# KLab/YAIK

Hardware: AMD Instinct MI355X
Metric: Mpix/s tile encode (alpha reject + 7 gradient passes + 8x8 range quant), 8K RGBA (higher is better)
Workload: dtype u8/int32 (+f32 mode-selection sums)

## Files before the change

yaik_amd/csrc/yk_encode2.hip:

```cpp
#include "yk_common.h"
#include "yk_curves.h"
#include "yk_device.h"
#include <mutex>

__constant__ float c_curve2[6][16] = YK_CURVE_TABLE;

#define LS YK_LSTRIDE
#ifdef YK_TEST_HOOKS
#define YK2_ABLATE(bit) ((P.ablate & (bit)) != 0)
#else
#define YK2_ABLATE(bit) false
#endif

__device__ __forceinline__ int y2_byte(uint32_t w, int ch) { return (w >> (8 * ch)) & 255; }
__device__ __forceinline__ uint32_t y2_absdiff(uint32_t a, uint32_t b) { uint32_t r; asm("v_sad_u32 %0, %1, %2, 0" : "=v"(r) : "v"(a), "v"(b)); return r; }
__device__ __forceinline__ int y2_round6(int v) { return (v & ~3) | (v >> 6); }
__device__ __forceinline__ int y2_round6p(int v) { v = min(v + 1, 255); return (v & ~3) | (v >> 6); }

typedef short y2s2 __attribute__((ext_vector_type(2)));
typedef unsigned short y2u2 __attribute__((ext_vector_type(2)));
__device__ __forceinline__ y2u2 y2_u2(uint32_t w) { return __builtin_bit_cast(y2u2, w); }
__device__ __forceinline__ y2s2 y2_s2(y2u2 v) { return __builtin_bit_cast(y2s2, v); }
__device__ __forceinline__ y2u2 y2_splat(int v) { const unsigned short t = (unsigned short)v; return (y2u2){ t, t }; }
__device__ __forceinline__ y2s2 y2_splats(int v) { const short t = (short)v; return (y2s2){ t, t }; }
// ... 377 lines not shown
    const int lane = pass.lane;
    const unsigned long long viable = y2_viable<SX, SY>(pass, cov) & ~evaluated;
    evaluated = 0ULL;
    if (viable == 0ULL) return;
    YK2_STAT(kPassId * 10 + 0, 1); YK2_STAT(kPassId * 10 + 8, __popcll(y2_spread<NX, NY>(viable)));
    if (y2_compact_sweep<SX, SY>(pass, viable, cov, evaluated)) return;
    const unsigned long long accept = y2_full_pass<SX, SY, SMOOTH>(pass, viable);
    if (accept == 0ULL) return;
    YK2_STAT(kPassId * 10 + 6, 1);
    y2_accept<SX, SY>(pass, cov, accept);
}

#define YK2_QROWS 258
#define YK2_QR0 32
#define YK2_QNR 224
#define YK2_QBYTES ((size_t)YK2_QNR * YK2_QROWS * 16)
#define YK2_RCPBYTES ((size_t)256 * sizeof(float))
#define YK2_DEFN1 224
#define YK2_DEFBYTES ((size_t)225 * YK2_DEFN1 * 4)
#define YK2_TABBYTES (YK2_QBYTES + YK2_RCPBYTES + YK2_DEFBYTES)
typedef _Float16 y2h2 __attribute__((ext_vector_type(2)));
__device__ __forceinline__ uint32_t y2_f16_bits(int n) { const _Float16 h = (_Float16)(float)n; return (uint32_t)__builtin_bit_cast(unsigned short, h); }
__global__ void yk_qtab_kernel(uint4* tab) {
    __shared__ int K[6][16];
    const int R = YK2_QR0 + (int)blockIdx.x, t = threadIdx.x;
    if (t < 96) { const int m = t >> 4, i = t & 15; K[m][i] = __float2int_rz(__fmul_rn(c_curve2[m][i], (float)R)); }
    __syncthreads();
    if (t < YK2_QROWS) {
        const int o = t - 2;
        uint32_t md[6], idx = 0;
        for (int m = 0; m < 6; m++) {
            const int cnt = m < 3 ? 16 : 8;
            int best = 1 << 30, bi = 0;
            for (int n = 0; n < cnt; n++) { const int d = abs(K[m][n] - o); if (d < best) { best = d; bi = n; } }
            best = min(best, 255);
            md[m] = y2_f16_bits(best);
            idx |= (uint32_t)bi << (4 * m);
        }
        tab[(size_t)blockIdx.x * YK2_QROWS + t] = make_uint4(md[0] | (md[1] << 16), md[2] | (md[3] << 16), md[4] | (md[5] << 16), idx);
    }
}
struct Y2TileDef { int base, BN, dist, R; };
__device__ __forceinline__ Y2TileDef y2_tile_def(const int min_, const int d8) {
    Y2TileDef d;
    d.base = (min_ * 63 + 112) / 224;
    d.BN = (d.base * 224) / 63;
    const int scale = 223 - d.BN;
    const int dnum = (d8 - 32) * 127 + (scale - 1);
    d.dist = (scale < 0) ? -dnum : dnum / scale;
    d.R = (d.dist * scale) / 127 + 32;
    return d;
}
__global__ void yk_deftab_kernel(uint32_t* tab) {
    const int min_ = blockIdx.x, d8 = 32 + (int)threadIdx.x;
    const Y2TileDef d = y2_tile_def(min_, d8);
    const int R = min(max(d.R, YK2_QR0), YK2_QR0 + YK2_QNR - 1);
    const uint32_t rowBase = (uint32_t)((R - YK2_QR0) * YK2_QROWS + 2 - d.BN + 256);
    tab[min_ * YK2_DEFN1 + (int)threadIdx.x] = rowBase | (((((uint32_t)d.dist & 255u) << 7) | ((uint32_t)d.base & 255u)) << 16);
}

__global__ void yk_selftest_qtab_kernel(const uint4* tab, const uint32_t* deftab, int* mismatches) {
    const int mn = blockIdx.x, mx = threadIdx.x;
    if (mx < mn) return;
    const int min_ = min(mn, 224);
    int diff = mx - min_; if (diff < 16) diff = 16;
    const int d8 = max(diff, 32);
    const Y2TileDef d = y2_tile_def(min_, d8);
    const int BN = d.BN, R = d.R;
    int bad = 0;
    if (R < YK2_QR0 || R >= YK2_QR0 + YK2_QNR || mn - BN < -2) { atomicAdd(mismatches, 1); return; }
    {
        const uint32_t e = deftab[min_ * YK2_DEFN1 + (d8 - 32)];
        if ((e & 0xFFFFu) != (uint32_t)((R - YK2_QR0) * YK2_QROWS + 2 - BN + 256)) bad++;
        if ((e >> 16) != ((((uint32_t)d.dist & 255u) << 7) | ((uint32_t)d.base & 255u))) bad++;
    }
    for (int m = 0; m < 6; m++) {
        const int cnt = m < 3 ? 16 : 8;
        int L[16];
        for (int i = 0; i < cnt; i++) {
            L[i] = __float2int_rz(__fadd_rn((float)BN, __fmul_rn(c_curve2[m][i], (float)R)));
            if (L[i] != BN + __float2int_rz(__fmul_rn(c_curve2[m][i], (float)R))) bad++;
        }
        for (int v = mn; v <= mx; v++) {
            int best = 1 << 30, bi = 0;
            for (int n = 0; n < cnt; n++) { const int dd = abs(L[n] - v); if (dd < best) { best = dd; bi = n; } }
            const uint4 row = tab[(size_t)(R - YK2_QR0) * YK2_QROWS + (v - BN + 2)];
            const uint32_t w = m < 2 ? row.x : (m < 4 ? row.y : row.z);
            const uint32_t hb = (m & 1) ? (w >> 16) : (w & 0xFFFFu);
            const int ix = (row.w >> (4 * m)) & 15;
            if (hb != y2_f16_bits(best) || ix != bi) bad++;
        }
    }
    if (bad) atomicAdd(mismatches, bad);
}

#define YK2_RUN 16
template <int K> __device__ __forceinline__ uint32_t y2_writelane_k(uint32_t v, uint32_t old) { asm("v_writelane_b32 %0, %1, %2" : "+v"(old) : "s"(v), "n"(K)); return old; }
__device__ __forceinline__ uint32_t y2_writelane(uint32_t v, int k, uint32_t old) {
    switch (k) {
        case 0: return y2_writelane_k<0>(v, old); case 1: return y2_writelane_k<1>(v, old); case 2: return y2_writelane_k<2>(v, old);
        case 3: return y2_writelane_k<3>(v, old); case 4: return y2_writelane_k<4>(v, old); case 5: return y2_writelane_k<5>(v, old);
        case 11: return y2_writelane_k<11>(v, old); default: return y2_writelane_k<12>(v, old);
    }
}
#ifdef YK2_TIMING
__device__ unsigned long long g_y2_times[65536 * 16];
#define YK2_PROBE(i) do { if ((i) == 0 && lane == 0 && unit < 65536) { g_y2_times[(size_t)unit * 16 + 10] = 0; g_y2_times[(size_t)unit * 16 + 11] = 0; g_y2_times[(size_t)unit * 16 + 12] = y2_t_entry; g_y2_times[(size_t)unit * 16 + 13] = ((unsigned long long)y2_xcc << 32) | y2_hwid; } if (lane == 0 && unit < 65536) { g_y2_times[(size_t)unit * 16 + 2 * (i)] = __builtin_amdgcn_s_memtime(); g_y2_times[(size_t)unit * 16 + 2 * (i) + 1] = __builtin_amdgcn_s_memrealtime(); } } while (0)
extern "C" int yk_debug_wave_times(unsigned long long* out) { return (int)hipMemcpyFromSymbol(out, HIP_SYMBOL(g_y2_times), sizeof(g_y2_times)); }
#else
#define YK2_PROBE(i) do { } while (0)
#endif
#define YK2_LUTW 84
#ifndef YK2_WIN
#define YK2_WIN 16
#endif
#ifndef YK2_PREF
#define YK2_PREF 8
#endif
#ifndef YK2_RVWIN
#define YK2_RVWIN 8
#endif

#define Y2_QUAD_X 0xB1
#define Y2_QUAD_Y 0x4E
template <int CTRL> __device__ __forceinline__ int y2_quad(int v) { return __builtin_amdgcn_update_dpp(v, v, CTRL, 0xF, 0xF, true); }
template <int CTRL> __device__ __forceinline__ float y2_quad(float v) { return __int_as_float(y2_quad<CTRL>(__float_as_int(v))); }
template <int FIRST> __device__ __forceinline__ void y2_quad_sums(float (&t)[6]) {
#define Y2_QX(i) "v_add_f32_dpp %" #i ", %" #i ", %" #i " quad_perm:[1,0,3,2] row_mask:0xf bank_mask:0xf\n\t"
#define Y2_QY(i) "v_add_f32_dpp %" #i ", %" #i ", %" #i " quad_perm:[2,3,0,1] row_mask:0xf bank_mask:0xf\n\t"
    if (FIRST == 0)
        asm volatile("s_nop 1\n\t" Y2_QX(0) Y2_QX(1) Y2_QX(2) Y2_QX(3) Y2_QX(4) Y2_QX(5) Y2_QY(0) Y2_QY(1) Y2_QY(2) Y2_QY(3) Y2_QY(4) Y2_QY(5)
                     : "+v"(t[0]), "+v"(t[1]), "+v"(t[2]), "+v"(t[3]), "+v"(t[4]), "+v"(t[5]));
    else
        asm volatile("s_nop 1\n\t" Y2_QX(0) Y2_QX(1) Y2_QX(2) Y2_QY(0) Y2_QY(1) Y2_QY(2) : "+v"(t[3]), "+v"(t[4]), "+v"(t[5]));
#undef Y2_QX
#undef Y2_QY
}
__device__ __forceinline__ float y2_row16_sum(float x) {
    x = __fadd_rn(x, y2_quad<Y2_QUAD_X>(x));
    x = __fadd_rn(x, y2_quad<Y2_QUAD_Y>(x));
    x = __fadd_rn(x, __int_as_float(__builtin_amdgcn_update_dpp(0, __float_as_int(x), 0x141, 0xF, 0xF, true)));
    x = __fadd_rn(x, __int_as_float(__builtin_amdgcn_update_dpp(0, __float_as_int(x), 0x140, 0xF, 0xF, true)));
    return x;
}
__device__ __forceinline__ uint32_t y2_byte_x4(uint32_t w, int ch) {
    uint32_t r; const uint32_t two = 2u;
    if (ch == 0) asm("v_lshlrev_b32_sdwa %0, %1, %2 dst_sel:DWORD dst_unused:UNUSED_PAD src0_sel:DWORD src1_sel:BYTE_0" : "=v"(r) : "v"(two), "v"(w));
    else if (ch == 1) asm("v_lshlrev_b32_sdwa %0, %1, %2 dst_sel:DWORD dst_unused:UNUSED_PAD src0_sel:DWORD src1_sel:BYTE_1" : "=v"(r) : "v"(two), "v"(w));
    else asm("v_lshlrev_b32_sdwa %0, %1, %2 dst_sel:DWORD dst_unused:UNUSED_PAD src0_sel:DWORD src1_sel:BYTE_2" : "=v"(r) : "v"(two), "v"(w));
    return r;
}
__device__ __forceinline__ void y2_fma_lo(float& acc, uint32_t h, float w) { asm volatile("v_fma_mix_f32 %0, %1, %2, %0 op_sel_hi:[1,0,0]" : "+v"(acc) : "v"(h), "v"(w)); }
__device__ __forceinline__ void y2_fma_hi(float& acc, uint32_t h, float w) { asm volatile("v_fma_mix_f32 %0, %1, %2, %0 op_sel:[1,0,0] op_sel_hi:[1,0,0]" : "+v"(acc) : "v"(h), "v"(w)); }
__device__ __forceinline__ uint32_t y2_pack3(int r, int g, int b) {
    return __builtin_amdgcn_perm((uint32_t)b, __builtin_amdgcn_perm((uint32_t)g, (uint32_t)r, 0x0C0C0400u), 0x0C040100u);
}

template <bool WANT_DST, bool MODE3>
__global__ __launch_bounds__(64, 4) void yk_encode2_kernel(const YkEncodeParams P) {
    constexpr int kStart = MODE3 ? 3 : 0;
    constexpr int kPixWords = 17 * LS, kLutWords = WANT_DST ? 16 * YK2_LUTW : 0;
    __shared__ __attribute__((aligned(16))) uint32_t s_mem[kPixWords > kLutWords ? kPixWords : kLutWords];
    uint32_t* const s_pix = s_mem;
    uint32_t (*const s_lut)[YK2_LUTW] = reinterpret_cast<uint32_t (*)[YK2_LUTW]>(s_mem);
    __shared__ uint32_t s_bm[24];
    __shared__ uint8_t s_list[64];
    __shared__ __attribute__((aligned(16))) float s_curve[WANT_DST ? 6 : 1][16];
    __shared__ __attribute__((aligned(16))) float s_rcp[256];
    __shared__ __attribute__((aligned(16))) uint32_t s_aux[432];
    uint32_t* const s_lat = s_aux;
    float (*const s_chain)[68] = reinterpret_cast<float (*)[68]>(s_aux);
    float* const s_err = reinterpret_cast<float*>(s_aux + 408);
    __shared__ uint32_t s_range[3 * 64];
    __shared__ __attribute__((aligned(16))) uint32_t s_sp[3 * 4 * 8 + 3 * 4 * 16];

    uint32_t* const s_tile = s_aux + 416;
    __shared__ uint32_t s_iwTest[WANT_DST ? 1024 : 1];
    uint32_t* const s_iw = WANT_DST ? s_iwTest : s_mem;
    uint32_t* const s_park = WANT_DST ? s_iwTest : s_sp;
    static_assert(WANT_DST || kPixWords >= 1024, "index words need 4 KB");

    const int lane = threadIdx.x;
    __builtin_amdgcn_s_setprio(3);
#ifdef YK2_TIMING
    const unsigned long long y2_t_entry = __builtin_amdgcn_s_memrealtime();
    const unsigned y2_hwid = __builtin_amdgcn_s_getreg((4 << 0) | (0 << 6) | (31 << 11)), y2_xcc = __builtin_amdgcn_s_getreg((20 << 0) | (0 << 6) | (31 << 11));
#endif
    typedef const __attribute__((address_space(4))) YkEncodeParams* Y2ParamPtr;
    auto strip = [&](const int slot, const int xcd, const int lane, Y2ParamPtr const Pp) {
    const __attribute__((address_space(4))) YkEncodeParams& P = *Pp;
    const int nBf = P.xBB64 * P.yBB64, nB = nBf * P.nFrames;
    const int grp = slot / (YK2_RUN * 4);
    const int unit = (grp * 8 + ((xcd + grp) & 7)) * (YK2_RUN * 4) + (slot - grp * (YK2_RUN * 4));
    int L = unit >> 2; const int wave = unit & 3;
    const bool spare = L >= nB;
    L = spare ? 0 : L;
    const uint32_t frU = yk_udiv((uint32_t)L, P.divNBf.mul, P.divNBf.shift);
    L -= (int)frU * nBf;
    const size_t fr = frU;
    const int32_t* const pl0 = P.plane[0] + fr * P.fs.plane; const int32_t* const pl1 = P.plane[1] + fr * P.fs.plane; const int32_t* const pl2 = P.plane[2] + fr * P.fs.plane;
    const int BY = (int)yk_udiv((uint32_t)L, P.divXBB64.mul, P.divXBB64.shift), BX = L - BY * P.xBB64;
    const int w = P.w, h = P.h;
    const int mt0 = (BY * 4 + wave) * P.mtW + BX * 4;

    YK2_PROBE(0);
    if (lane < 24) s_bm[lane] = 0;
    typedef uint32_t y2_u32x2 __attribute__((ext_vector_type(2)));
    typedef int32_t y2_i32x4 __attribute__((ext_vector_type(4)));
    y2_u32x2 keep8; y2_i32x4 bnd;
    {
        const int g4 = (lane & 15) * 4, r0 = lane >> 4;
        const int gx = BX * 64 + g4;
        const bool inX = gx + 3 < w;
        const int gxc = min(gx, w - 4);
        const int gyS = BY * 64 + wave * 16;
        const int gyB = min(gyS, P.hAvail - 1);
        const size_t rowBase = (size_t)gyB * (size_t)P.strideElems;
        const char* const b0 = reinterpret_cast<const char*>(pl0 + rowBase);
        const char* const b1 = reinterpret_cast<const char*>(pl1 + rowBase);
        const char* const b2 = reinterpret_cast<const char*>(pl2 + rowBase);
        int4 R[4], G[4], B[4];
#pragma unroll
        for (int k = 0; k < 4; k++) {
            const int rel = min(gyS + r0 + 4 * k, P.hAvail - 1) - gyB;
            const uint32_t off = (uint32_t)(rel * P.strideElems + gxc) * 4u;
            R[k] = *reinterpret_cast<const int4*>(b0 + off);
            G[k] = *reinterpret_cast<const int4*>(b1 + off);
            B[k] = *reinterpret_cast<const int4*>(b2 + off);
        }
        int4 Rb, Gb, Bb;
        {
            const int rel = min(gyS + 16, P.hAvail - 1) - gyB;
            const uint32_t off = (uint32_t)(rel * P.strideElems + gxc) * 4u;
            Rb = *reinterpret_cast<const int4*>(b0 + off);
            Gb = *reinterpret_cast<const int4*>(b1 + off);
            Bb = *reinterpret_cast<const int4*>(b2 + off);
        }
        uint32_t hcol;
        const int hr = min(max(lane - 32, 0), 16);
        {
            const int rel = min(gyS + hr, P.hAvail - 1) - gyB;
            const uint32_t off = (uint32_t)(rel * P.strideElems + min(BX * 64 + 64, w - 1)) * 4u;
            hcol = y2_pack3(*reinterpret_cast<const int32_t*>(b0 + off), *reinterpret_cast<const int32_t*>(b1 + off), *reinterpret_cast<const int32_t*>(b2 + off));
        }
        const float4 rc4 = *reinterpret_cast<const float4*>(P.qtab + YK2_QBYTES + (size_t)lane * 16);
        const uint4* const orow = P.outTab + (wave * YK2_OT_ROWS + (lane & (YK2_OT_ROWS - 1))) * 2;
        const uint4 ta = orow[0], tb = orow[1];
        {
            const bool rowIn = BY * 64 + wave * 16 < h;
            const uintptr_t args = reinterpret_cast<uintptr_t>(Pp);
            const uintptr_t kpIn = reinterpret_cast<uintptr_t>(P.keep) + fr * P.fs.keep + (uintptr_t)(mt0 & ~3);
            const uintptr_t bpIn = reinterpret_cast<uintptr_t>(P.bounds) + fr * 64;
            const uintptr_t kp = (P.keep != nullptr && rowIn) ? kpIn : args, bp = P.bounds != nullptr ? bpIn : args;
            asm volatile("s_load_dwordx2 %0, %2, 0x0\n\ts_load_dwordx4 %1, %3, 0x0" : "=&s"(keep8), "=&s"(bnd) : "s"(kp), "s"(bp));
        }

        __builtin_amdgcn_s_setprio(0);
        if (spare) return;
        {
            const uint32_t frT = frU + P.outFrame0;
            const uint32_t o = ta.x + frT * ta.y + (uint32_t)BX * ta.z + (uint32_t)BY * ta.w;
            s_park[lane] = ((uint32_t)BX < tb.x && (uint32_t)BY < tb.y) ? o : YK2_OT_NONE;
            s_park[64 + lane] = tb.z;
        }
        uint4 o[4], ob;
#pragma unroll
        for (int k = 0; k < 4; k++) {
            o[k] = make_uint4(y2_pack3(R[k].x, G[k].x, B[k].x), y2_pack3(R[k].y, G[k].y, B[k].y), y2_pack3(R[k].z, G[k].z, B[k].z), y2_pack3(R[k].w, G[k].w, B[k].w));
            *reinterpret_cast<uint4*>(&s_pix[(r0 + 4 * k) * LS + g4]) = o[k];
        }
        ob = make_uint4(y2_pack3(Rb.x, Gb.x, Bb.x), y2_pack3(Rb.y, Gb.y, Bb.y), y2_pack3(Rb.z, Gb.z, Bb.z), y2_pack3(Rb.w, Gb.w, Bb.w));
        if (lane < 16) *reinterpret_cast<uint4*>(&s_pix[16 * LS + g4]) = ob;
        if (BX * 64 + 64 > w) {
            if (!inX) {
#pragma unroll
                for (int k = 0; k < 4; k++) *reinterpret_cast<uint4*>(&s_pix[(r0 + 4 * k) * LS + g4]) = make_uint4(o[k].w, o[k].w, o[k].w, o[k].w);
                if (lane < 16) *reinterpret_cast<uint4*>(&s_pix[16 * LS + g4]) = make_uint4(ob.w, ob.w, ob.w, ob.w);
            }
        }
        if (lane >= 32 && lane <= 48) s_pix[hr * LS + 64] = hcol;
        *reinterpret_cast<float4*>(&s_rcp[lane * 4]) = rc4;

    }
    asm volatile("s_waitcnt lgkmcnt(0)" : "+s"(keep8), "+s"(bnd));
    __syncthreads();
    YK2_PROBE(1);

    const int q = lane >> 4, cx = y2_cell_x(lane & 15), cy = y2_cell_y(lane & 15);
    const int bxCell = q * 16 + cx * 4, byCell = wave * 16 + cy * 4;
    const int gxCell = BX * 64 + bxCell, gyCell = BY * 64 + byCell;
    const int lcell = (cy * 4) * LS + bxCell;
    const int lat = cy * 17 + q * 4 + cx;
    const bool mtIn = (BX * 64 + q * 16 < w) && (BY * 64 + wave * 16 < h);

    uint32_t pw[16];
#pragma unroll
    for (int r = 0; r < 4; r++) {
        const uint4 t = *reinterpret_cast<const uint4*>(&s_pix[lcell + r * LS]);
        pw[r * 4 + 0] = t.x; pw[r * 4 + 1] = t.y; pw[r * 4 + 2] = t.z; pw[r * 4 + 3] = t.w;
    }

    unsigned long long cov = 0ULL;
    unsigned long long evaluated = 0ULL;
    {
        bool dead = !mtIn;
        {
            const int lim = 4 * P.rejectFactor + 1;
            const y2u2 rb0 = y2_u2(pw[0] & 0x00FF00FFu), rb1 = y2_u2(pw[1] & 0x00FF00FFu), rb2 = y2_u2(pw[2] & 0x00FF00FFu), rb3 = y2_u2(pw[3] & 0x00FF00FFu);
            const y2u2 ga = y2_u2(__builtin_amdgcn_perm(pw[1], pw[0], 0x0C050C01u)), gb = y2_u2(__builtin_amdgcn_perm(pw[2], pw[1], 0x0C050C01u)),
                       gc = y2_u2(__builtin_amdgcn_perm(pw[3], pw[2], 0x0C050C01u));
            const y2u2 l2 = y2_splat(lim);
            const y2u2 u1 = rb0 + rb2 - rb1 - rb1 + l2, u2 = rb1 + rb3 - rb2 - rb2 + l2, ug = ga + gc - gb - gb + l2;
            const y2u2 um = __builtin_elementwise_max(__builtin_elementwise_max(u1, u2), ug);
            dead |= __builtin_bit_cast(uint32_t, __builtin_elementwise_sub_sat(um, y2_splat(2 * lim))) != 0u;
        }
        const unsigned long long deadLanes = __ballot(dead);
        YK2_STAT(75, 1); YK2_STAT(76, ~deadLanes == 0ULL ? 1 : 0); YK2_STAT(77, __popcll(deadLanes));
        const bool stripInside = (BX * 64 + 64 <= w) && (BY * 64 + wave * 16 + 16 <= h);
        if (~deadLanes != 0ULL && !YK2_ABLATE(2)) {
            auto latticePoint = [&](const int idx) {
                const int lr = (idx * 241) >> 12, lc = idx - lr * 17;
                const uint32_t raw = s_pix[(lr * 4) * LS + lc * 4];
                const uint32_t r6 = (raw & 0x00FCFCFCu) | ((raw >> 6) & 0x00030303u);
                const uint32_t z = (raw & 0x007F7F7Fu) + 0x00010101u;
                const uint32_t inc = (z ^ (raw & 0x00808080u)) | (((z & raw & 0x00808080u) >> 7) * 255u);
                const uint32_t p6 = (inc & 0x00FCFCFCu) | ((inc >> 6) & 0x00030303u);
                s_lat[0 * YK2_LATN + idx] = __builtin_amdgcn_perm(r6, raw, 0x0C040C00u);
                s_lat[1 * YK2_LATN + idx] = __builtin_amdgcn_perm(r6, raw, 0x0C050C01u);
                s_lat[2 * YK2_LATN + idx] = __builtin_amdgcn_perm(r6, raw, 0x0C060C02u);
                s_lat[3 * YK2_LATN + idx] = __builtin_amdgcn_perm(p6, p6, 0x0C010C00u);
                s_lat[4 * YK2_LATN + idx] = __builtin_amdgcn_perm(p6, p6, 0x0C020C02u);
            };
            latticePoint(lane);
            if (lane < YK2_LATN - 64) latticePoint(lane + 64);
            __syncthreads();
            y2s2 rg[16], bb[8];
#pragma unroll
            for (int k = 0; k < 16; k++) rg[k] = y2_rg(pw[k]);
#pragma unroll
            for (int k = 0; k < 8; k++) bb[k] = y2_bb(pw[2 * k], pw[2 * k + 1]);
            const Y2Pass S = { s_lat, lat, cx, cy, rg, bb, deadLanes, stripInside, gxCell, gyCell, w, h, P.rejectFactor, s_bm, bxCell, byCell, s_pix, s_list, s_range, lane };
            if (deadLanes == 0ULL) y2_grad_pass<4, 4, true>(S, cov, evaluated);
            else y2_grad_pass<4, 4>(S, cov, evaluated);
            if (~(cov | deadLanes) != 0ULL) {
                y2_grad_pass<4, 3>(S, cov, evaluated);
                y2_grad_pass<3, 4>(S, cov, evaluated);
                y2_grad_pass<3, 3>(S, cov, evaluated);
                y2_grad_pass<3, 2>(S, cov, evaluated);
                y2_grad_pass<2, 3>(S, cov, evaluated);
                y2_grad_pass<2, 2>(S, cov, evaluated);
            }
#pragma unroll
            for (int r = 0; r < 4; r++) {
                const uint4 t = *reinterpret_cast<const uint4*>(&s_pix[lcell + r * LS]);
                pw[r * 4 + 0] = t.x; pw[r * 4 + 1] = t.y; pw[r * 4 + 2] = t.z; pw[r * 4 + 3] = t.w;
            }
        }
    }
    const int mtIdx = mt0 + q;
    __syncthreads();
    YK2_PROBE(2);
    uint8_t* const small = P.small;
    const uint32_t tabOff = s_park[lane], tabSel = s_park[64 + lane];
    const uint32_t tabVal = (s_bm[tabSel & 31u] >> ((tabSel >> 8) & 31u)) & (~0u >> (tabSel >> 16));
    uint32_t off32 = (uint32_t)lane - 8u < 5u ? tabOff : ~0u;
    uint32_t val32 = (uint32_t)lane - 8u < 3u ? tabVal : 0u;
    {
        if ((uint32_t)lane - 1u < 3u) *(small + tabOff) = (uint8_t)tabVal;
        const unsigned long long t = ((cov >> 2) ^ cov) & 0x0C0C0C0C0C0C0C0CULL;
        const unsigned long long covRM = cov ^ t ^ (t << 2);
        uint32_t off16 = ((lane & 15) == 0 && mtIn) ? P.oCov + (frU * (uint32_t)P.fs.coverage + (uint32_t)mtIdx) * 2u : ~0u;
        uint32_t val16 = (uint32_t)((covRM >> (q * 16)) & 0xFFFFULL);
        if ((uint32_t)lane - 4u < 3u) { off16 = tabOff; val16 = tabVal; }
        if (off16 != ~0u) *reinterpret_cast<uint16_t*>(small + off16) = (uint16_t)val16;
        if (P.pixCache != nullptr) {
            const bool cellIn = (gxCell < w) && (gyCell < h);
            if (cellIn && !((cov >> lane) & 1ULL)) {
                const uint32_t strip = (uint32_t)((BY * 4 + wave) * P.xBB64 + BX);
                uint4* dstp = P.pixCache + (size_t)strip * 256 + lane;
#pragma unroll
                for (int r = 0; r < 4; r++) dstp[r * 64] = make_uint4(pw[r * 4 + 0], pw[r * 4 + 1], pw[r * 4 + 2], pw[r * 4 + 3]);
            }
        }
    }
    YK2_PROBE(3);
    int cxB = 0, cyB = 0, cw = w, chh = P.fullH, discard = 1;
    if (P.bounds != nullptr) {
        const int b0 = bnd.x, b1 = bnd.y, b2 = bnd.z, b3 = bnd.w;
        discard = (b0 == 0 && b1 == 0 && b2 == w && b3 == P.fullH) ? 1 : 0;
        cxB = (b0 >> 3) << 3; cyB = (b1 >> 3) << 3;
        cw = (((b2 + 7) >> 3) << 3) - cxB; chh = (((b3 + 7) >> 3) << 3) - cyB;
    }
    const int cxl = cx & 1, cyl = cy & 1;
    const int tgx = gxCell - cxl * 4, tgyl = gyCell - cyl * 4, tgy = tgyl + P.y0;
    const bool tileIn = (tgx + 8 <= w) && (tgyl + 8 <= h);
    const bool part = tileIn && tgx >= cxB && tgx < cxB + cw && tgy >= cyB && tgy < cyB + chh && (tgx + 8 <= cw) && (tgy + 8 <= chh);
    const uint32_t keep4 = (uint32_t)((((unsigned long long)keep8.y << 32) | keep8.x) >> (8 * (mt0 & 3)));
    const bool keepMT = (P.keep == nullptr) || discard || (mtIn && ((keep4 >> (8 * q)) & 0xFFu) != 0u);
    const bool tileLive = part && keepMT;
    const int l00 = lane & ~3;
    const uint32_t quadN = (uint32_t)((~cov) >> l00) & 15u;
    const int v00 = (int)(quadN & 1u), v01 = (int)((quadN >> 2) & 1u);
    const bool valid = tileLive && ((quadN >> (lane & 3)) & 1u);
    const int nTop = __popc(quadN & 3u), nBot = __popc(quadN >> 2);
    const int tileIdx = (tgyl >> 3) * P.tilesW + (tgx >> 3);
    const size_t T8 = (size_t)P.tilesW * P.tilesH;
    const int tw = lane >> 2;
    const bool writer = ((lane & 3) == 0) && tileIn;
    const unsigned long long validMask = __ballot(valid);
    const bool fullTiles = !WANT_DST && __ballot(tileLive && quadN != 15u && quadN != 0u) == 0ULL;

    {
        const int n16 = (tileLive && !YK2_ABLATE(1)) ? (nTop + nBot) : 0;
        if ((P.tilesW & 7) == 0) {
            if (validMask != 0ULL) {
#pragma unroll
                for (int r = 0; r < 2; r++) {
                    const bool mine = writer && ((cy >> 1) == r);
                    const unsigned long long b0 = __ballot(mine && (n16 & 1)), b1 = __ballot(mine && (n16 & 2)), b2 = __ballot(mine && (n16 & 4));
                    const unsigned long long bd = __ballot(mine && n16 > 0);
                    val32 = y2_writelane((uint32_t)(__popcll(b0) + 2 * __popcll(b1) + 4 * __popcll(b2)) | ((uint32_t)__popcll(bd) << 16), 11 + r, val32);
                }
            }
        } else if (writer && n16 > 0) {
            uint32_t* const blockCntP = P.blockCnt + fr * P.fs.blockN;
            atomicAdd(&blockCntP[((size_t)tileIdx >> 10) * 2], 16u * (uint32_t)n16);
            atomicAdd(&blockCntP[((size_t)tileIdx >> 10) * 2 + 1], 1u);
        }
        if (off32 != ~0u) *reinterpret_cast<uint32_t*>(small + off32) = val32;
    }

    YK2_STAT(70, validMask != 0ULL ? 1 : 0); YK2_STAT(74, __popcll(validMask));
    { const int nv = __popcll(validMask); YK2_STAT(120 + (nv == 0 ? 0 : nv <= 4 ? 1 : nv <= 8 ? 2 : nv <= 16 ? 3 : nv <= 32 ? 4 : nv < 64 ? 5 : 6), 1); (void)nv; }
    uint32_t defs01 = 0u, defs2c = 0u;
    if (validMask != 0ULL && !YK2_ABLATE(1)) {
        uint8_t* const slotsP = P.slots + fr * P.fs.slots;
        uint32_t* lut = &s_lut[WANT_DST ? tw : 0][0];
        if (WANT_DST) {
            s_curve[lane >> 4][lane & 15] = c_curve2[lane >> 4][lane & 15];
            if (lane < 32) s_curve[4 + (lane >> 4)][lane & 15] = c_curve2[4 + (lane >> 4)][lane & 15];
        }
        const int j4 = lane & 3;
        const int nValidLanes = __popcll(validMask);
        const bool spread = nValidLanes <= 4 && !WANT_DST;
        const int vRank = (int)__builtin_amdgcn_mbcnt_hi((uint32_t)(validMask >> 32), __builtin_amdgcn_mbcnt_lo((uint32_t)validMask, 0u));
        uint32_t slotOff[4];
#pragma unroll
        for (int r = 0; r < 4; r++) {
            const int yIn = cyl * 4 + r;
            const int pos = (yIn < 4) ? (yIn * 4 * nTop + (cxl ? 4 * v00 : 0))
                                      : (16 * nTop + (yIn - 4) * 4 * nBot + (cxl ? 4 * v01 : 0));
            slotOff[r] = (uint32_t)tileIdx * (uint32_t)YK_SLOT + (uint32_t)(pos >> 1);
        }
        int tmn[3], tmx[3];
        {
            y2u2 mnRB = y2_splat(0xFFFF), mxRB = y2_splat(0), mnG = y2_splat(0xFFFF), mxG = y2_splat(0);
            if (valid) {
#pragma unroll
                for (int k = 0; k < 16; k += 2) {
                    const y2u2 a = y2_u2(pw[k] & 0x00FF00FFu), b = y2_u2(pw[k + 1] & 0x00FF00FFu), g = y2_u2(__builtin_amdgcn_perm(pw[k + 1], pw[k], 0x0C050C01u));
                    if (k == 0) { mnRB = __builtin_elementwise_min(a, b); mxRB = __builtin_elementwise_max(a, b); mnG = g; mxG = g; }
                    else {
                        mnRB = __builtin_elementwise_min(__builtin_elementwise_min(mnRB, a), b); mxRB = __builtin_elementwise_max(__builtin_elementwise_max(mxRB, a), b);
                        mnG = __builtin_elementwise_min(mnG, g); mxG = __builtin_elementwise_max(mxG, g);
                    }
                }
            }
            tmn[0] = (int)mnRB.x; tmn[2] = (int)mnRB.y; tmx[0] = (int)mxRB.x; tmx[2] = (int)mxRB.y;
            tmn[1] = min((int)mnG.x, (int)mnG.y); tmx[1] = max((int)mxG.x, (int)mxG.y);
#pragma unroll
            for (int p = 0; p < 3; p++) {
                tmn[p] = min(tmn[p], y2_quad<Y2_QUAD_X>(tmn[p])); tmx[p] = max(tmx[p], y2_quad<Y2_QUAD_X>(tmx[p]));
                tmn[p] = min(tmn[p], y2_quad<Y2_QUAD_Y>(tmn[p])); tmx[p] = max(tmx[p], y2_quad<Y2_QUAD_Y>(tmx[p]));
            }
        }
        const uint32_t* const defTab = reinterpret_cast<const uint32_t*>(P.qtab + YK2_QBYTES + YK2_RCPBYTES);
        uint32_t tdef[3];
#pragma unroll
        for (int p = 0; p < 3; p++) {
            const int none = tmn[p] > 255;
            const int mn = none ? 0 : tmn[p], mx = none ? 0 : tmx[p];
            const int min_ = min(mn, 224);
            const int d8 = max(mx - min_, 32);
            tdef[p] = defTab[(uint32_t)(min_ * YK2_DEFN1 + d8 - 32)];
            s_range[p * 64 + lane] = (uint32_t)mn | ((uint32_t)mx << 8);
        }
        const uint8_t* const qrows = P.qtab - (size_t)256 * 16;
        if (spread && !YK2_ABLATE(4)) {
            if (valid) s_list[vRank] = (uint8_t)lane;
            __builtin_amdgcn_fence(__ATOMIC_RELEASE, "wavefront"); __builtin_amdgcn_wave_barrier(); __builtin_amdgcn_fence(__ATOMIC_ACQUIRE, "wavefront");
            const int spI = lane >> 4, spK = lane & 15;
            const bool spAct = spI < nValidLanes;
            const int spSrc = (int)s_list[spAct ? spI : 0];
            const int sq = spSrc >> 4, scx = y2_cell_x(spSrc & 15), scy = y2_cell_y(spSrc & 15);
            const uint32_t spx = s_pix[(scy * 4 + (spK >> 2)) * LS + sq * 16 + scx * 4 + (spK & 3)];
#pragma unroll
            for (int p = 0; p < 3; p++) {
                const uint32_t q16s = (uint32_t)__builtin_amdgcn_ds_bpermute(spSrc << 2, (int)((tdef[p] & 0xFFFFu) << 4));
                float t6[6] = { 0.0f, 0.0f, 0.0f, 0.0f, 0.0f, 0.0f };
                if (spAct) {
                    const uint32_t v4 = y2_byte_x4(spx, p);
                    const uint4 row = *reinterpret_cast<const uint4*>(qrows + (size_t)((v4 << 2) + q16s));
                    const float rv = *reinterpret_cast<const float*>(reinterpret_cast<const char*>(s_rcp) + v4);
                    if (!MODE3) { y2_fma_lo(t6[0], row.x, rv); y2_fma_hi(t6[1], row.x, rv); y2_fma_lo(t6[2], row.y, rv); }
                    y2_fma_hi(t6[3], row.y, rv); y2_fma_lo(t6[4], row.z, rv); y2_fma_hi(t6[5], row.z, rv);
                    s_sp[96 + (p * 4 + spI) * 16 + spK] = row.w;
                }
#pragma unroll
                for (int m = kStart; m < 6; m++) {
                    const float tot = y2_row16_sum(t6[m]);
                    if (spK == 0) s_sp[(p * 4 + spI) * 8 + m] = __float_as_uint(tot);
                }
            }
            __builtin_amdgcn_fence(__ATOMIC_RELEASE, "wavefront"); __builtin_amdgcn_wave_barrier(); __builtin_amdgcn_fence(__ATOMIC_ACQUIRE, "wavefront");
        }
        uint4 win[16];
        auto issueRows = [&](const int pl, const int k0, const int k1) {
            if (valid && !spread && !YK2_ABLATE(4)) {
                const uint32_t q16 = (tdef[pl] & 0xFFFFu) << 4;
                {
#pragma unroll
                    for (int k = k0; k < k1; k++) {
                        const uint32_t v4 = y2_byte_x4(pw[k], pl);
                        win[k] = *reinterpret_cast<const uint4*>(qrows + (size_t)((v4 << 2) + q16));
                    }
                }
            }
        };
        issueRows(0, 0, YK2_PREF);
#pragma unroll
        for (int p = 0; p < 3; p++) {
            const uint32_t qrow16 = (tdef[p] & 0xFFFFu) << 4;
            float sm[6] = { 0.0f, 0.0f, 0.0f, 0.0f, 0.0f, 0.0f };
            issueRows(p, YK2_PREF, 16);
            if (valid && !spread && !YK2_ABLATE(4)) {
                float rvw[YK2_RVWIN];
                auto issueRcp = [&](const int k, float& rv) { rv = *reinterpret_cast<const float*>(reinterpret_cast<const char*>(s_rcp) + y2_byte_x4(pw[k], p)); };
#pragma unroll
                for (int k = 0; k < YK2_RVWIN; k++) issueRcp(k, rvw[k]);
#pragma unroll
                for (int k = 0; k < 16; k++) {
                    __builtin_amdgcn_sched_barrier(0);
                    const uint4 row = win[k]; const float rv = rvw[k % YK2_RVWIN];
                    if (!MODE3) { y2_fma_lo(sm[0], row.x, rv); y2_fma_hi(sm[1], row.x, rv); y2_fma_lo(sm[2], row.y, rv); }
                    y2_fma_hi(sm[3], row.y, rv); y2_fma_lo(sm[4], row.z, rv); y2_fma_hi(sm[5], row.z, rv);
                    s_iw[k * 64 + lane] = row.w;
                    if (k + YK2_RVWIN < 16) issueRcp(k + YK2_RVWIN, rvw[k % YK2_RVWIN]);
                }
                __builtin_amdgcn_sched_barrier(0);
            }
            if (spread && valid && !YK2_ABLATE(4)) {
#pragma unroll
                for (int m = kStart; m < 6; m++) sm[m] = __uint_as_float(s_sp[(p * 4 + vRank) * 8 + m]);
#pragma unroll
                for (int k4 = 0; k4 < 4; k4++) {
                    const uint4 iw4 = *reinterpret_cast<const uint4*>(&s_sp[96 + (p * 4 + vRank) * 16 + k4 * 4]);
                    s_iw[(k4 * 4 + 0) * 64 + lane] = iw4.x; s_iw[(k4 * 4 + 1) * 64 + lane] = iw4.y; s_iw[(k4 * 4 + 2) * 64 + lane] = iw4.z; s_iw[(k4 * 4 + 3) * 64 + lane] = iw4.w;
                }
            }
            if (p < 2) issueRows(p + 1, 0, YK2_PREF);
            float tm[6] = { sm[0], sm[1], sm[2], sm[3], sm[4], sm[5] };
            y2_quad_sums<kStart>(tm);
            int bestMode = kStart; float bestT = tm[kStart];
            bool near = false;
#pragma unroll
            for (int m = kStart + 1; m < 6; m++) {
                const float t = tm[m];
                const float lo = fminf(t, bestT), hi = fmaxf(t, bestT);
                near |= !(__fmul_rn(lo, 1.00002f) < hi);
                bestMode = (t <= bestT) ? m : bestMode;
                bestT = lo;
            }
            bool amb = false;
            uint32_t ties = 0;
            if (__ballot(near && tileLive) != 0ULL) {
                int bm = kStart; float bt = tm[kStart];
#pragma unroll
                for (int m = kStart + 1; m < 6; m++) {
                    const float t = tm[m];
                    const float lo = fminf(t, bt), hi = fmaxf(t, bt);
                    const bool eq = (t == bt);
                    amb |= !eq && !(__fmul_rn(lo, 1.00002f) < hi);
                    if (eq && t != 0.0f) ties |= (1u << m) | ((uint32_t)bm << (8 + 3 * m));
                    bm = (t <= bt) ? m : bm;
                    bt = lo;
                }
            }
            if (__ballot(ties != 0u && tileLive) != 0ULL) {
                YK2_STAT(73, 1);
                const uint32_t tr = s_range[p * 64 + lane];
                const uint32_t mn = tr & 255u, mx = tr >> 8;
                const uint32_t va = min(mn + (uint32_t)j4, mx), vb = min(mn + 4u + (uint32_t)j4, mx);
                const uint4 ra = *reinterpret_cast<const uint4*>(qrows + (size_t)((va << 4) + qrow16));
                const uint4 rb = *reinterpret_cast<const uint4*>(qrows + (size_t)((vb << 4) + qrow16));
                const uint32_t rxa = __builtin_amdgcn_alignbit(ra.x, ra.x, 16), rya = __builtin_amdgcn_alignbit(ra.y, ra.y, 16), rza = __builtin_amdgcn_alignbit(ra.z, ra.z, 16);
                const uint32_t rxb = __builtin_amdgcn_alignbit(rb.x, rb.x, 16), ryb = __builtin_amdgcn_alignbit(rb.y, rb.y, 16), rzb = __builtin_amdgcn_alignbit(rb.z, rb.z, 16);
                uint32_t acc[9] = { (ra.x ^ rxa) | (rb.x ^ rxb),
                                    (ra.y ^ rya) | (rb.y ^ ryb),
                                    (ra.z ^ rza) | (rb.z ^ rzb),
                                    (ra.x ^ ra.y) | (rb.x ^ rb.y),
                                    (ra.x ^ ra.z) | (rb.x ^ rb.z),
                                    (ra.y ^ ra.z) | (rb.y ^ rb.z),
                                    (ra.x ^ rya) | (rb.x ^ ryb),
                                    (ra.x ^ rza) | (rb.x ^ rzb),
                                    (ra.y ^ rza) | (rb.y ^ rzb) };
#pragma unroll
                for (int i = 0; i < 9; i++) { acc[i] |= (uint32_t)y2_quad<Y2_QUAD_X>((int)acc[i]); acc[i] |= (uint32_t)y2_quad<Y2_QUAD_Y>((int)acc[i]); }
                bool differ = (mx - mn) > 7u;
                auto pairDiffers = [&](const int i, const int j) -> bool {
                    const int lo = i < j ? i : j, hi = i < j ? j : i;
                    if (lo == 0 && hi == 1) return (acc[0] & 0xFFFFu) != 0u;
                    if (lo == 2 && hi == 3) return (acc[1] & 0xFFFFu) != 0u;
                    if (lo == 4 && hi == 5) return (acc[2] & 0xFFFFu) != 0u;
                    if (lo == 0 && hi == 2) return (acc[3] & 0xFFFFu) != 0u;
                    if (lo == 1 && hi == 3) return (acc[3] >> 16) != 0u;
                    if (lo == 0 && hi == 4) return (acc[4] & 0xFFFFu) != 0u;
                    if (lo == 1 && hi == 5) return (acc[4] >> 16) != 0u;
                    if (lo == 2 && hi == 4) return (acc[5] & 0xFFFFu) != 0u;
                    if (lo == 3 && hi == 5) return (acc[5] >> 16) != 0u;
                    if (lo == 0 && hi == 3) return (acc[6] & 0xFFFFu) != 0u;
                    if (lo == 1 && hi == 2) return (acc[6] >> 16) != 0u;
                    if (lo == 0 && hi == 5) return (acc[7] & 0xFFFFu) != 0u;
                    if (lo == 1 && hi == 4) return (acc[7] >> 16) != 0u;
                    if (lo == 2 && hi == 5) return (acc[8] & 0xFFFFu) != 0u;
                    return (acc[8] >> 16) != 0u;
                };
#pragma unroll
                for (int m = kStart + 1; m < 6; m++) {
                    const uint32_t fb = ((ties >> m) & 1u) ? ((ties >> (8 + 3 * m)) & 7u) : 7u;
#pragma unroll
                    for (int b2 = kStart; b2 < m; b2++) differ |= (fb == (uint32_t)b2) && pairDiffers(b2, m);
                }
                if (ties != 0u && differ) amb = true;
            }
            uint32_t cLo = 0, cHi = 0;
            if (valid) {
                const uint32_t sh = 4u * (uint32_t)bestMode;
#pragma unroll
                for (int k = 0; k < 16; k++) {
                    const uint32_t code = s_iw[k * 64 + lane] >> sh;
                    if (k < 8) cLo = __builtin_amdgcn_alignbit(code, cLo, 4); else cHi = __builtin_amdgcn_alignbit(code, cHi, 4);
                }
            }
            if (YK2_ABLATE(16)) amb = true;
            unsigned long long ambMask = __ballot(amb && tileLive);
            YK2_STAT(72, __popcll(ambMask) / 4); YK2_STAT(71, ambMask != 0ULL ? 1 : 0);
#ifdef YK2_TIMING
            if (lane == 0 && unit < 65536 && ambMask) { g_y2_times[(size_t)unit * 16 + 10] += (unsigned long long)__popcll(ambMask) / 4; g_y2_times[(size_t)unit * 16 + 11] += 1; }
#endif
            if (WANT_DST) {
                const int rowBase = (int)(tdef[p] & 0xFFFFu) - 256 - 2;
                const int base = (int)((tdef[p] >> 16) & 127u);
                const int BN = (base * 224) / 63;
                const int rangeDecode = (rowBase + BN) / YK2_QROWS + YK2_QR0;
                const float Rf = (float)rangeDecode, BNf = (float)BN;
#pragma unroll
                for (int m = 0; m < 3; m++) {
                    uint32_t Lq[4];
#pragma unroll
                    for (int k = 0; k < 4; k++)
                        Lq[k] = (uint32_t)__float2int_rz(__fadd_rn(BNf, __fmul_rn(s_curve[m][j4 * 4 + k], Rf)));
                    *reinterpret_cast<uint4*>(&lut[m * 20 + j4 * 4]) = make_uint4(Lq[0] << 8, Lq[1] << 8, Lq[2] << 8, Lq[3] << 8);
                }
#pragma unroll
                for (int m = 3; m < 6; m++) {
                    uint32_t Lq[2];
#pragma unroll
                    for (int k = 0; k < 2; k++)
                        Lq[k] = (uint32_t)__float2int_rz(__fadd_rn(BNf, __fmul_rn(s_curve[m][j4 * 2 + k], Rf)));
                    *reinterpret_cast<uint2*>(&lut[60 + (m - 3) * 8 + j4 * 2]) = make_uint2(Lq[0] << 8, Lq[1] << 8);
                }
                __builtin_amdgcn_fence(__ATOMIC_RELEASE, "wavefront");
                __builtin_amdgcn_wave_barrier();
                __builtin_amdgcn_fence(__ATOMIC_ACQUIRE, "wavefront");
            }
            while (ambMask != 0ULL) {
                const int a00 = (__ffsll((long long)ambMask) - 1) & ~3;
                ambMask &= ~(0xFULL << a00);
                if (l00 == a00) {
#pragma unroll
                    for (int r = 0; r < 4; r++) {
                        const uint32_t kSel = 0x0C0C0000u | ((4u + (uint32_t)p) << 8) | (uint32_t)p;
                        const uint32_t lo2 = __builtin_amdgcn_perm(pw[r * 4 + 1], pw[r * 4 + 0], kSel), hi2 = __builtin_amdgcn_perm(pw[r * 4 + 3], pw[r * 4 + 2], kSel);
                        s_tile[(cyl * 4 + r) * 2 + cxl] = __builtin_amdgcn_perm(hi2, lo2, 0x05040100u);
                    }
                }
                const uint32_t tq16 = (uint32_t)__builtin_amdgcn_readlane((int)qrow16, a00), tqn = (uint32_t)__builtin_amdgcn_readlane((int)quadN, a00);
                __builtin_amdgcn_fence(__ATOMIC_RELEASE, "wavefront");
                __builtin_amdgcn_wave_barrier();
                __builtin_amdgcn_fence(__ATOMIC_ACQUIRE, "wavefront");
                {
                    const uint32_t v = (uint32_t)reinterpret_cast<const uint8_t*>(s_tile)[lane];
                    const bool pv = ((tqn >> (((lane >> 5) << 1) | ((lane >> 2) & 1))) & 1u) != 0u;
                    uint4 rw = make_uint4(0u, 0u, 0u, 0u);
                    if (pv) rw = *reinterpret_cast<const uint4*>(qrows + (size_t)((v << 4) + tq16));
                    const float fv = (float)v, rr = pv ? s_rcp[v] : 0.0f;
                    const y2h2 h01 = __builtin_bit_cast(y2h2, rw.x), h23 = __builtin_bit_cast(y2h2, rw.y), h45 = __builtin_bit_cast(y2h2, rw.z);
                    s_chain[0][lane] = yk_div_exact((float)h01.x, fv, rr);
                    s_chain[1][lane] = yk_div_exact((float)h01.y, fv, rr);
                    s_chain[2][lane] = yk_div_exact((float)h23.x, fv, rr);
                    s_chain[3][lane] = yk_div_exact((float)h23.y, fv, rr);
                    s_chain[4][lane] = yk_div_exact((float)h45.x, fv, rr);
                    s_chain[5][lane] = yk_div_exact((float)h45.y, fv, rr);
                }
                __builtin_amdgcn_fence(__ATOMIC_RELEASE, "wavefront");
                __builtin_amdgcn_wave_barrier();
                __builtin_amdgcn_fence(__ATOMIC_ACQUIRE, "wavefront");
                if (lane < 6 && lane >= kStart) {
                    float sacc = 0.0f;
                    const float4* cp = reinterpret_cast<const float4*>(&s_chain[lane][0]);
#pragma unroll
                    for (int k = 0; k < 16; k++) {
                        const float4 a = cp[k];
                        sacc = __fadd_rn(__fadd_rn(__fadd_rn(__fadd_rn(sacc, a.x), a.y), a.z), a.w);
                    }
                    s_err[lane] = sacc;
                }
                __builtin_amdgcn_fence(__ATOMIC_RELEASE, "wavefront");
                __builtin_amdgcn_wave_barrier();
                __builtin_amdgcn_fence(__ATOMIC_ACQUIRE, "wavefront");
                if (l00 == a00) {
                    bestMode = -1; float bestErr = 99999999.0f;
                    for (int m = kStart; m < 6; m++) {
                        const float e = s_err[m];
                        if (e <= bestErr) { bestErr = e; bestMode = m; }
                    }
                    if (valid) {
                        const uint32_t sh = 4u * (uint32_t)bestMode;
#pragma unroll
                        for (int k = 0; k < 16; k++) {
                            const uint32_t code = s_iw[k * 64 + lane] >> sh;
                            if (k < 8) cLo = __builtin_amdgcn_alignbit(code, cLo, 4); else cHi = __builtin_amdgcn_alignbit(code, cHi, 4);
                        }
                    }
                }
// ... 92 lines not shown
```

Measured before the change: 242,700.

## Early-exit fully covered strips and defer pixel reload until needed

After the gradient passes, the kernel now computes wave-uniform masks for in-bounds cells, uncovered cells and kept macro-tiles. If no uncovered, kept cell remains, it writes the small header word, zeroes the tile-info entries and returns, skipping the quantization stage. The LDS reload of pixels after the passes happens only when the data will be coded or cached, with an empty asm marking the registers as clobbered so the compiler does not keep them live. Keep-mask evaluation becomes bit tricks plus an inverse ballot; this adds a new early-return path that must exactly replicate the side effects of the full path.

Measured after the change: 244,600 (median of 2 runs). No clear change (+0.8%).

```diff
diff --git a/yaik_amd/csrc/yk_encode2.hip b/yaik_amd/csrc/yk_encode2.hip
--- a/yaik_amd/csrc/yk_encode2.hip
+++ b/yaik_amd/csrc/yk_encode2.hip
@@ -703,6 +703,7 @@
 
     unsigned long long cov = 0ULL;
     unsigned long long evaluated = 0ULL;
+    bool passesRan = false;
     {
         bool dead = !mtIn;
         {
@@ -751,11 +752,9 @@
                 y2_grad_pass<2, 3>(S, cov, evaluated);
                 y2_grad_pass<2, 2>(S, cov, evaluated);
             }
-#pragma unroll
-            for (int r = 0; r < 4; r++) {
-                const uint4 t = *reinterpret_cast<const uint4*>(&s_pix[lcell + r * LS]);
-                pw[r * 4 + 0] = t.x; pw[r * 4 + 1] = t.y; pw[r * 4 + 2] = t.z; pw[r * 4 + 3] = t.w;
-            }
+            passesRan = true;
+            asm("" : "=v"(pw[0]), "=v"(pw[1]), "=v"(pw[2]), "=v"(pw[3]), "=v"(pw[4]), "=v"(pw[5]), "=v"(pw[6]), "=v"(pw[7]),
+                     "=v"(pw[8]), "=v"(pw[9]), "=v"(pw[10]), "=v"(pw[11]), "=v"(pw[12]), "=v"(pw[13]), "=v"(pw[14]), "=v"(pw[15]));
         }
     }
     const int mtIdx = mt0 + q;
@@ -774,9 +773,41 @@
         uint32_t val16 = (uint32_t)((covRM >> (q * 16)) & 0xFFFFULL);
         if ((uint32_t)lane - 4u < 3u) { off16 = tabOff; val16 = tabVal; }
         if (off16 != ~0u) *reinterpret_cast<uint16_t*>(small + off16) = (uint16_t)val16;
-        if (P.pixCache != nullptr) {
-            const bool cellIn = (gxCell < w) && (gyCell < h);
-            if (cellIn && !((cov >> lane) & 1ULL)) {
+    }
+    const int discard = (P.bounds == nullptr || (bnd.x == 0 && bnd.y == 0 && bnd.z == w && bnd.w == P.fullH)) ? 1 : 0;
+    unsigned long long inMask = ~0ULL;
+    if (!((BX * 64 + 64 <= w) && (BY * 64 + wave * 16 + 16 <= h))) {
+        const int nC = min(max((w - BX * 64) >> 3, 0), 8), nR = min(max((h - BY * 64 - wave * 16) >> 3, 0), 2);
+        const int lim = 16 * (nC >> 1) + 4 * (nC & 1);
+        const unsigned long long top = (lim != 0 && nR != 0) ? (0x00FF00FF00FF00FFULL & (~0ULL >> (64 - lim))) : 0ULL;
+        inMask = top | (nR == 2 ? top << 8 : 0ULL);
+    }
+    const unsigned long long uncov = ~cov & inMask;
+    unsigned long long keptLanes = ~0ULL;
+    if (P.keep != nullptr && !discard) {
+        const uint32_t keep4 = (uint32_t)((((unsigned long long)keep8.y << 32) | keep8.x) >> (8 * (mt0 & 3)));
+        const uint32_t nz = ((((keep4 & 0x7F7F7F7Fu) + 0x7F7F7F7Fu) | keep4) >> 7) & 0x01010101u;
+        const uint32_t lo = ((nz & 1u) | ((nz << 8) & 0x10000u)) * 0xFFFFu, hi = (((nz >> 16) & 1u) | ((nz >> 8) & 0x10000u)) * 0xFFFFu;
+        keptLanes = ((unsigned long long)hi << 32) | lo;
+    }
+    const bool toCode = (uncov & keptLanes) != 0ULL;
+    const bool toCache = P.pixCache != nullptr && uncov != 0ULL;
+#ifdef YK2_STATS
+    if (!toCode) {
+        const unsigned long long keptIn = keptLanes & inMask;
+        YK2_STAT(160, 1); YK2_STAT(uncov == 0ULL ? 161 : keptIn == 0ULL ? 162 : 163, 1); YK2_STAT(165, toCache ? 1 : 0);
+    }
+#endif
+    if (toCode || toCache) {
+        if (passesRan) {
+#pragma unroll
+            for (int r = 0; r < 4; r++) {
+                const uint4 t = *reinterpret_cast<const uint4*>(&s_pix[lcell + r * LS]);
+                pw[r * 4 + 0] = t.x; pw[r * 4 + 1] = t.y; pw[r * 4 + 2] = t.z; pw[r * 4 + 3] = t.w;
+            }
+        }
+        if (toCache) {
+            if (__builtin_amdgcn_inverse_ballot_w64(uncov)) {
                 const uint32_t strip = (uint32_t)((BY * 4 + wave) * P.xBB64 + BX);
                 uint4* dstp = P.pixCache + (size_t)strip * 256 + lane;
 #pragma unroll
@@ -785,10 +816,21 @@
         }
     }
     YK2_PROBE(3);
-    int cxB = 0, cyB = 0, cw = w, chh = P.fullH, discard = 1;
+    if (!toCode) {
+        if (off32 != ~0u) *reinterpret_cast<uint32_t*>(small + off32) = val32;
+        YK2_STAT(120, 1);
+        if (__builtin_amdgcn_inverse_ballot_w64(inMask & 0x1111111111111111ULL)) {
+            const uint32_t base = P.oInfo + (frU * (uint32_t)P.fs.tileInfo + (uint32_t)((BY * 4 + wave) * 2 * P.tilesW + BX * 8)) * 8u;
+            const uint32_t tcol = (((uint32_t)lane >> 3) & 6u) | (((uint32_t)lane >> 2) & 1u);
+            const uint32_t offI = base + (((lane & 8) ? (uint32_t)P.tilesW : 0u) + tcol) * 8u;
+            *reinterpret_cast<uint2*>(small + offI) = make_uint2(0u, 0u);
+        }
+        YK2_PROBE(4);
+        return;
+    }
+    int cxB = 0, cyB = 0, cw = w, chh = P.fullH;
     if (P.bounds != nullptr) {
         const int b0 = bnd.x, b1 = bnd.y, b2 = bnd.z, b3 = bnd.w;
-        discard = (b0 == 0 && b1 == 0 && b2 == w && b3 == P.fullH) ? 1 : 0;
         cxB = (b0 >> 3) << 3; cyB = (b1 >> 3) << 3;
         cw = (((b2 + 7) >> 3) << 3) - cxB; chh = (((b3 + 7) >> 3) << 3) - cyB;
     }
@@ -796,8 +838,7 @@
     const int tgx = gxCell - cxl * 4, tgyl = gyCell - cyl * 4, tgy = tgyl + P.y0;
     const bool tileIn = (tgx + 8 <= w) && (tgyl + 8 <= h);
     const bool part = tileIn && tgx >= cxB && tgx < cxB + cw && tgy >= cyB && tgy < cyB + chh && (tgx + 8 <= cw) && (tgy + 8 <= chh);
-    const uint32_t keep4 = (uint32_t)((((unsigned long long)keep8.y << 32) | keep8.x) >> (8 * (mt0 & 3)));
-    const bool keepMT = (P.keep == nullptr) || discard || (mtIn && ((keep4 >> (8 * q)) & 0xFFu) != 0u);
+    const bool keepMT = __builtin_amdgcn_inverse_ballot_w64(keptLanes);
     const bool tileLive = part && keepMT;
     const int l00 = lane & ~3;
     const uint32_t quadN = (uint32_t)((~cov) >> l00) & 15u;
@@ -832,6 +873,7 @@
     }
 
     YK2_STAT(70, validMask != 0ULL ? 1 : 0); YK2_STAT(74, __popcll(validMask));
+    YK2_STAT(164, validMask == 0ULL ? 1 : 0);
     { const int nv = __popcll(validMask); YK2_STAT(120 + (nv == 0 ? 0 : nv <= 4 ? 1 : nv <= 8 ? 2 : nv <= 16 ? 3 : nv <= 32 ? 4 : nv < 64 ? 5 : 6), 1); (void)nv; }
     uint32_t defs01 = 0u, defs2c = 0u;
     if (validMask != 0ULL && !YK2_ABLATE(1)) {
```
